# qiyueyao/Kubernetes-verification

Hardware: AMD Instinct MI355X
Metric: pod-pairs/sec for reachability build + all-checks latency, 100k pods, 1/2/4/8 GPU (higher is better)
Workload: dtype u64

## Files before the change

kubernetes-verification_amd/csrc/kano_engine.hpp:

```cpp
#pragma once
#include <hip/hip_runtime.h>
#include <hip/hip_ext.h>

#include <algorithm>
#include <cmath>
#include <functional>
#include <cerrno>
#include <cstdint>
#include <cstdlib>
#include <cstring>
#include <string>
#include <vector>
#include <array>
#include <chrono>
#include <ctime>
#include <cstdio>
#include <dlfcn.h>
#include <link.h>
#include <thread>

#include "kano_hip.h"
#include "kano_internal.hpp"
#include "kano_prims.hpp"

// ... 94 lines not shown
  DBuf mct;
  bool shg_prefilled = false;
  i64 dx_ldY = 0, dx_PBo = 0;
  bool dense_sel = false;
  int ac_lds = 1;
  int mlists_side_ok = 1;
  bool mlists_side = false;
  bool rin_marked = false;
  i64 sel_early_cap = -1;
  int path_lds = 1;
  int rows_ch = ROWS_CH;
  int rows_cww = MAX_CWW_KNOB;
  int impact_form = 0;
  int shadow_r = 0;
  int shg_sub_lds = 1;
  int rows_cu_off = 20;
  int xcd_split = 1;
  i64 xcd_min_bytes = XCD_MIN_BYTES;
  int xcd_write = XCD_WRITE;
  int xcd_eng0 = -1;
  bool xcd_tried = false, eng_on_xcd = false, xcd_last_ok = false;
  int side_mode = 0;
  int xcd_side = -1;
  hipStream_t stream_x = nullptr, stream2_x = nullptr, stream3x = nullptr;
  hipStream_t stream2_u = nullptr;
  hipEvent_t ev_sw = nullptr, ev_sw2 = nullptr;
  i64 rows_cu_bytes = 8ll << 30;
  int num_cus = 0, rows_cus = 0;

  ClassSet rc, cc;
// ... 21 lines not shown
  hipEvent_t ev_pre = nullptr, ev_pre_done = nullptr, ev_pre_ac = nullptr;
  bool pre_forked = false, pre_side_pending = false, pre_ac_pending = false;
  bool tail_compacted = false;
  hipEvent_t ev_pairs = nullptr;
  DBuf gid, gids, cgroup, R, multi, A1, A2, own, cross, gmin, gmax, ckey, corder, kcnt, koff;
  DBuf flags, T, loff, L, tp, poff, out, tcnt, toff;
  DBuf scratch_words, ident;
  DBuf xw, xg;
  i64 xg_emul = -1;
  DBuf pT, pR[2], pD[2], pA, pB, pcnt;
  DBuf xv, asel, aalw, iterm, idead, irows;
  i64 inc_A = 0, inc_acap = 0, inc_xcols = 0;
  std::vector<uint8_t> dead;
  bool user_edited = false;
  i64 shadow_total = -1;
  DBuf conflict_out;
  i64 conflict_total = -1;
  DBuf impact_out, impact_ess;
  float impact_ms = 0.f;
  bool vs_count_only = false;
  bool shg_ran = false;
  DBuf shg_h, shg_tkey, shg_trep, shg_slot, shg_isrep, shg_gidx, shg_gid, shg_reps, shg_sub,
      shg_err;
  DBuf sizes;
  DBuf icnt, ioff, sysrow, idxd;
  u64* ghost = nullptr;
  void* row_stage = nullptr;
  u64* gmirror = nullptr;
  u64* gmirror_dev = nullptr;
  DBuf sig_ctr;
// ... 32 lines not shown
  bool priming = false;
  bool consume_prime = false;
  bool prime_pre_marked = false;
  bool prime_alist_valid = false;
  u64 prime_sig = 0;
  u64* bell = nullptr;
  u64* bell_dev = nullptr;
  u64 bell_seq = 0;
  u64 gate_ticks = 0;
  u64 wall_khz = 100000;
  DBuf gate_wait;
  u64 gate_seq0 = 0;
  u64 gate_forced = 0;
  DBuf sizes_alt;
  hipEvent_t ev_tail = nullptr;
  hipEvent_t ev_rt[2][2] = {};
  bool rows_time_pending[2] = {false, false};
  hipEvent_t ev_m0 = nullptr, ev_m1 = nullptr;
  bool mfma_time_pending = false;
  double mfma_ops_last = 0.0, mfma_ops_sum = 0.0, mfma_ms_sum = 0.0;
  i64 mfma_n = 0;
  float rows_ms_last = 0.f;
  double rows_ms_sum = 0.0, rows_ms_min = 0.0, rows_ms_max = 0.0;
  i64 rows_ms_n = 0;
  bool vs_open = false, vs_shadow = false, vs_cross_want = false, vs_cross_on = false;
  bool vs_have_sys = false, vs_sys_on = false;
  bool vs_rows = false;
  i64 vs_nb = 0, vs_rl = 0;
};

// ... 46 lines not shown
```

kubernetes-verification_amd/csrc/kano_hip.hip:

```cpp
#include "kano_engine.hpp"
#include "kano_kernels.hpp"

namespace kano_eng {

int fail(kano_ctx* ctx, int code, const std::string& msg) {
  ctx->err = msg;
  return code;
}

int settle(kano_ctx* ctx);

int dalloc(kano_ctx* ctx, DBuf& b, size_t bytes) {
  if (bytes == 0) bytes = 16;
  if (b.p && b.bytes >= bytes) return 0;
  if (b.p) {
    KTRY(settle(ctx));
    KCHK(hipFree(b.p));
    b.p = nullptr;
    b.bytes = 0;
  }
  const hipError_t e = hipMalloc(&b.p, bytes);
  if (e != hipSuccess) {
    b.p = nullptr;
    return fail(ctx, -ENOMEM, "hipMalloc(" + std::to_string(bytes) + " bytes) -> " +
// ... 229 lines not shown
  std::swap(ctx->aloff, a.aloff);
  std::swap(ctx->alist, a.alist);
  std::swap(ctx->alcoff, a.alcoff);
  std::swap(ctx->alc, a.alc);
  std::swap(ctx->rc.moff, a.rmoff);
  std::swap(ctx->rc.mem, a.rmem);
  std::swap(ctx->cc.moff, a.cmoff);
  std::swap(ctx->cc.mem, a.cmem);
  std::swap(ctx->cc.cls, a.ccls);
  std::swap(ctx->hflag, a.hflag);
  std::swap(ctx->hlist, a.hlist);
  std::swap(ctx->Mc, a.Mc);
  ctx->rows_set ^= 1;
}

void ring_bell(kano_ctx* ctx) {
  if (ctx->bell) __atomic_store_n(ctx->bell, ctx->bell_seq, __ATOMIC_SEQ_CST);
}

int unprime(kano_ctx* ctx) {
  if (!ctx->primed || ctx->priming) return 0;
  ctx->primed = false;
  ring_bell(ctx);
  ctx->gate_forced = ctx->bell_seq;
  KCHK(hipStreamSynchronize(ctx->stream));
  KCHK(hipStreamSynchronize(ctx->stream2));
  std::swap(ctx->sizes, ctx->sizes_alt);
  swap_rows_ptrs(ctx);
  ctx->alist_valid = ctx->prime_alist_valid;
  return 0;
// ... 62 lines not shown
  KCHK(hipEventElapsedTime(&ms, ctx->ev_m0, ctx->ev_m1));
  ctx->mfma_ms_sum += ms;
  ctx->mfma_ops_sum += ctx->mfma_ops_last;
  ctx->mfma_n += 1;
  return 0;
}

int read_slots(kano_ctx* ctx, int first, int count, i64* out) {
  KCHK(hipMemcpyAsync(ctx->ghost, P_<u64>(ctx->sizes) + first, sizeof(u64) * count,
                      hipMemcpyDeviceToHost, ctx->stream));
  KTRY(sync(ctx));
  for (int k = 0; k < count; ++k) out[k] = (i64)ctx->ghost[k];
  return 0;
}

void* pinned_dev(void* host) {
  if (!host || (reinterpret_cast<uintptr_t>(host) & 15)) return nullptr;
  hipPointerAttribute_t at{};
  void* dptr = nullptr;
  if (hipPointerGetAttributes(&at, host) == hipSuccess && at.type == hipMemoryTypeHost &&
      at.devicePointer)
    dptr = at.devicePointer;
  (void)hipGetLastError();
  return dptr;
}

int copy_out(kano_ctx* ctx, void* host, const void* dev, size_t bytes, hipStream_t st) {
  if (bytes == 0) return 0;
  hipPointerAttribute_t at{};
  void* dptr = nullptr;
  if (hipPointerGetAttributes(&at, host) == hipSuccess && at.type == hipMemoryTypeHost &&
      at.devicePointer)
// ... 306 lines not shown

int sel_spb(const kano_ctx* ctx) {
  return ctx->P >= 8 * std::max<i64>(1, ctx->rc.U) ? TPB : WPB;
}

int front_fills(kano_ctx* ctx, FillBatch& fb) {
  KTRY(dalloc(ctx, ctx->sizes, sizeof(u64) * SZ_SLOTS));
  KTRY(fb.add(ctx->sizes, sizeof(u64) * SZ_SLOTS, 0u));
  KTRY(classify_alloc1(ctx, ctx->rc, fb));
  KTRY(classify_alloc1(ctx, ctx->cc, fb));
  return 0;
}

int select_engine_streams(kano_ctx* ctx);

int front_a(kano_ctx* ctx) {
  KTRY(select_engine_streams(ctx));
  ctx->rc.m0 = ctx->r0;
  ctx->rc.m1 = ctx->r1;
  ctx->cc.m0 = 0;
  ctx->cc.m1 = ctx->n;
  {
    FillBatch fb(ctx);
    KTRY(front_fills(ctx, fb));
    KTRY(fb.run());
  }
  KTRY(classify_phase1(ctx));
  KTRY(mirror_begin(ctx));
  ctx->mlists_side = ctx->stream2 != nullptr && ctx->mlists_side_ok;
  if (!ctx->mlists_side && ctx->stream2) {
    KTRY(classify_phase2a(ctx));
    KCHK(hipEventRecord(ctx->ev_pre, ctx->stream));
    return 0;
  }
  return classify_phase2a(ctx);
}

// ... 1061 lines not shown
        if (k == "packed") ctx->cls_packed = v;
        if (k == "rw" && v >= 0 && v <= 2) ctx->rows_wide = v;
        if (k == "rwg" && v >= 0) ctx->rows_w_grid = v;
        if (k == "rheavy" && v >= 0 && v <= 2) ctx->rows_early_heavy = v;
        if (k == "aipt" && v >= 0 && v <= ASSIGN_IPT) ctx->assign_ipt = v;
        if (k == "sww" && v >= 1 && v <= SORT_LDS_WW) ctx->sort_ww = v;
        if (k == "cww" && v >= 16 && v <= MAX_CWW_KNOB && v % 16 == 0) ctx->rows_cww = v;
        if (k == "rch" && v >= 1 && v <= 1024) ctx->rows_ch = v;
        if (k == "async") ctx->async_rows = v;
        if (k == "shcount" && v >= 0 && v <= 2) ctx->shadow_count_mode = v;
        if (k == "pathdens" && v >= 0 && v <= 101) ctx->path_dens = v;
        if (k == "pathtm" && (v == 1 || v == 2 || v == 4)) ctx->path_tm = v;
        if (k == "pathlds") ctx->path_lds = v;
        if (k == "pathtn" && (v == 2 || v == 4)) ctx->path_tn = v;
        if (k == "shgsub") ctx->shg_sub_lds = v;
        if (k == "impf" && v >= 0 && v <= 2) ctx->impact_form = v;
        if (k == "shr" && (v == 1 || v == 2 || v == 4 || v == 8)) ctx->shadow_r = v;
        if (k == "rcu" && v >= 0 && v <= 28 && (v < 4 || v % 4 == 0)) ctx->rows_cu_off = v;
        if (k == "rcubytes" && v >= 0) ctx->rows_cu_bytes = (i64)v << 30;
        if (k == "xcd") ctx->xcd_split = v;
        if (k == "xcdmin" && v >= 0) ctx->xcd_min_bytes = (i64)v << 10;
        if (k == "xcdw" && v >= 1 && v <= 7) ctx->xcd_write = v;
        if (k == "xcde" && v >= 0 && v <= 7) ctx->xcd_eng0 = v;
        if (k == "xcdside" && v >= -1 && v <= 1) ctx->xcd_side = v;
        if (k == "hgemm" && (v == -1 || v == 0 || v == 22 || v == 42 || v == 44))
          ctx->heavy_gemm = v;
        if (k == "hgemmmin" && v > 0) ctx->heavy_gemm_min = v;
        if (k == "hortime") ctx->time_or = v;
        if (k == "hexplds" && v >= 2 && v <= 4) ctx->heavy_expand_lds = v;
        if (k == "dx") ctx->dx_on = v;
// ... 33 lines not shown
                              hipFuncAttributeMaxDynamicSharedMemorySize,
                              (int)sizeof(u64) * MAX_CWW_KNOB);
  }
  mark("func_attributes");
  if (hipStreamCreateWithFlags(&ctx->stream3, hipStreamNonBlocking) != hipSuccess) {
    ctx->stream3 = nullptr;
    kano_destroy(ctx);
    return -EIO;
  }
  if (!g_create_lean) KTRY(ensure_masked_stream(ctx));
  mark("write_streams");
  if (hipStreamCreateWithPriority(&ctx->stream2, hipStreamNonBlocking, prio_main) != hipSuccess ||
      hipEventCreateWithFlags(&ctx->ev_fork, hipEventDisableTiming) != hipSuccess ||
      hipEventCreateWithFlags(&ctx->ev_sizes, hipEventDisableTiming) != hipSuccess ||
      hipEventCreateWithFlags(&ctx->ev_tail, hipEventDisableTiming) != hipSuccess ||
      hipEventCreateWithFlags(&ctx->ev_rin, hipEventDisableTiming) != hipSuccess ||
      hipEventCreateWithFlags(&ctx->ev_rin_e, hipEventDisableTiming) != hipSuccess ||
      hipEventCreateWithFlags(&ctx->ev_fork2, hipEventDisableTiming) != hipSuccess ||
      hipEventCreateWithFlags(&ctx->ev_join2, hipEventDisableTiming) != hipSuccess ||
      hipEventCreateWithFlags(&ctx->ev_pre, hipEventDisableTiming) != hipSuccess ||
      hipEventCreateWithFlags(&ctx->ev_pre_done, hipEventDisableTiming) != hipSuccess ||
      hipEventCreateWithFlags(&ctx->ev_pre_ac, hipEventDisableTiming) != hipSuccess ||
      hipEventCreateWithFlags(&ctx->ev_sw, hipEventDisableTiming) != hipSuccess ||
      hipEventCreateWithFlags(&ctx->ev_sw2, hipEventDisableTiming) != hipSuccess ||
      hipEventCreateWithFlags(&ctx->ev_pairs, hipEventDisableTiming) != hipSuccess ||
      hipEventCreate(&ctx->ev_m0) != hipSuccess || hipEventCreate(&ctx->ev_m1) != hipSuccess ||
      hipEventCreateWithFlags(&ctx->ev_rows_end[0], hipEventDisableTiming) != hipSuccess ||
      hipEventCreateWithFlags(&ctx->ev_rows_end[1], hipEventDisableTiming) != hipSuccess ||
      hipEventCreate(&ctx->ev_rt[0][0]) != hipSuccess || hipEventCreate(&ctx->ev_rt[0][1]) != hipSuccess ||
      hipEventCreate(&ctx->ev_rt[1][0]) != hipSuccess || hipEventCreate(&ctx->ev_rt[1][1]) != hipSuccess) {
    kano_destroy(ctx);
// ... 95 lines not shown
  RowsInputs& ra = ctx->rin_alt;
  for (DBuf* b : {&ra.wioff, &ra.wicls, &ra.soffc, &ra.slist, &ra.aloff, &ra.alist, &ra.alcoff,
                  &ra.alc, &ra.rmoff, &ra.rmem, &ra.cmoff, &ra.cmem, &ra.ccls, &ra.hflag,
                  &ra.hlist, &ra.Mc})
    dfree(*b);
  for (auto& e : ctx->ev)
    if (e) (void)hipEventDestroy(e);
  if (ctx->own_stream && ctx->stream) (void)hipStreamDestroy(ctx->stream);
  if (ctx->stream2) (void)hipStreamDestroy(ctx->stream2);
  if (ctx->stream3) (void)hipStreamDestroy(ctx->stream3);
  if (ctx->stream3m) (void)hipStreamDestroy(ctx->stream3m);
  for (hipStream_t t : {ctx->stream_x, ctx->stream2_x, ctx->stream3x, ctx->stream2_u})
    if (t) (void)hipStreamDestroy(t);
  for (hipEvent_t e : {ctx->ev_sw, ctx->ev_sw2})
    if (e) (void)hipEventDestroy(e);
  for (hipEvent_t e : {ctx->ev_fork, ctx->ev_tail, ctx->ev_rin, ctx->ev_rin_e, ctx->ev_sizes,
                       ctx->ev_fork2, ctx->ev_join2, ctx->ev_pre, ctx->ev_pre_done, ctx->ev_pre_ac, ctx->ev_pairs, ctx->ev_m0, ctx->ev_m1, ctx->ev_rows_end[0],
                       ctx->ev_rows_end[1], ctx->ev_rt[0][0], ctx->ev_rt[0][1], ctx->ev_rt[1][0],
                       ctx->ev_rt[1][1]})
    if (e) (void)hipEventDestroy(e);
  delete ctx;
}

const char* kano_last_error(const kano_ctx* ctx) { return ctx ? ctx->err.c_str() : "null context"; }

int kano_set_stream(kano_ctx* ctx, void* s) {
  if (!ctx) return -EINVAL;
  KCHK(hipSetDevice(ctx->device));
  KTRY(settle(ctx));
  KTRY(leave_xcd_streams(ctx));
  KCHK(hipStreamSynchronize(ctx->stream2));
// ... 292 lines not shown
               const PreRun& pre_run = PreRun()) {
  if (!ctx) return -EINVAL;
  const bool consume = ctx->primed && ctx->consume_prime;
  ctx->consume_prime = false;
  if (!consume) KTRY(unprime(ctx));
  if (!ctx->have_pods || !ctx->have_pols) return fail(ctx, -EINVAL, "kano_build: inputs not set");
  if (path < 0 || path > 2) return fail(ctx, -EINVAL, "kano_build: unknown path");
  KCHK(hipSetDevice(ctx->device));
  ctx->built = false;
  ctx->rows_deferred = false;
  ctx->lists_mode = false;
  ctx->rows_timed = false;
  ctx->rows_dirty = false;
  ctx->cols_valid = false;
  ctx->shadow_total = -1;
  ctx->conflict_total = -1;
  ctx->sig_armed = 0;
  ctx->sel_early_cap = -1;
  ctx->shg_prefilled = false;
  const i64 rl = rows_local(ctx);
  if (!ctx->defer_alloc)
    KTRY(dalloc(ctx, ctx->M, sizeof(u64) * std::max<i64>(1, rl * ctx->ldM)));
  KTRY(dalloc(ctx, ctx->color, sizeof(u64) * ctx->ldM));
  KTRY(dalloc(ctx, ctx->colnand, sizeof(u64) * ctx->ldM));
  KTRY(stage_mark(ctx, 0, ctx->stream));
  KTRY(do_front(ctx, path, consume));
  KTRY(mirror_begin(ctx));
  KTRY(do_back_pre(ctx, pre_fill, pre_run));
  KTRY(sel_place_early(ctx));
  KTRY(read_sizes(ctx));
// ... 474 lines not shown
  if (nt > 0 && nl > 0) {
    hipLaunchKernelGGL(k_shadow_compact, dim3((unsigned)nt), dim3(TPB), 0, st,
                       P_<i64>(ctx->soffc), U, P_<int32_t>(ctx->slist), P_<i64>(ctx->pfoff),
                       P_<uint8_t>(ctx->flags), nf, P_<i64>(ctx->toff), P_<int2>(ctx->L), nl);
    KLAUNCH();
  }
  if (rl > 0 && total > 0) {
    hipLaunchKernelGGL(k_shadow_emit, dim3(nblk(rl)), dim3(TPB), 0, st,
                       P_<int32_t>(ctx->rc.cls), ctx->r0, ctx->r1, P_<i64>(ctx->loff),
                       P_<int2>(ctx->L), P_<i64>(ctx->poff), P_<int2>(ctx->out), total,
                       (const i64*)nullptr, nl);
    KLAUNCH();
  }
  KTRY(stage_mark(ctx, 6, st));
  ctx->shadow_total = total;
  return 0;
}

}

extern "C" {

int kano_shadow(kano_ctx* ctx, int64_t* count) {
  KTRY(ensure_built(ctx));
  ctx->vs_count_only = false;
  KTRY(shadow_front(ctx));
  i64 tot[2] = {0, 0};
  KTRY(read_slots(ctx, SZ_NL, 2, tot));
  KTRY(shadow_back(ctx, tot[0], tot[1]));
  if (count) *count = tot[1];
  return 0;
}

int kano_shadow_fetch(kano_ctx* ctx, int32_t* pairs) {
  KTRY(ensure_built(ctx));
  if (ctx->shadow_total < 0) return fail(ctx, -EINVAL, "kano_shadow_fetch before kano_shadow");
  if (ctx->shadow_total > 0) {
    if (!pairs) return fail(ctx, -EINVAL, "kano_shadow_fetch: NULL buffer");
    KCHK(hipMemcpyAsync(pairs, ctx->out.p, sizeof(int2) * ctx->shadow_total,
                        hipMemcpyDeviceToHost, ctx->stream));
  }
  return sync(ctx);
}

}

namespace {
int lists_setup(kano_ctx* ctx, const char* what, int64_t n_lists, int64_t nbits, int64_t P,
                const int64_t* soff, const int32_t* slist, const uint64_t* allow_rows) {
  if (!ctx) return -EINVAL;
  if (n_lists < 0 || nbits < 0 || P < 0 || !soff || n_lists >= (int64_t)INT32_MAX / 2)
    return fail(ctx, -EINVAL, std::string(what) + ": bad arguments");
  KCHK(hipSetDevice(ctx->device));
  KTRY(settle(ctx));
  const i64 nnz = soff[n_lists];
  for (i64 e = 0; e < nnz; ++e)
    if (slist[e] < 0 || slist[e] >= P)
      return fail(ctx, -ERANGE, std::string(what) + ": policy index out of range");
  ctx->conflict_total = -1;
  ctx->built = false;
  ctx->lists_mode = true;
  ctx->n = nbits;
  ctx->W = (nbits + 63) / 64;
  ctx->ldM = std::max<i64>(2, (ctx->W + 1) & ~(i64)1);
  ctx->P = P;
  ctx->PB = (P + 63) / 64;
  ctx->r0 = 0;
  ctx->r1 = n_lists;
  ctx->nnz_sel = nnz;
// ... 67 lines not shown
  return kano_shadow(ctx, count);
}

int kano_conflict(kano_ctx* ctx, int* raises) {
  KTRY(ensure_built(ctx));
  if (!raises) return fail(ctx, -EINVAL, "kano_conflict: NULL");
  *raises = ctx->max_sel >= 2 ? 1 : 0;
  return 0;
}

}

namespace {
int conflict_front(kano_ctx* ctx, bool count_only, i64* nl, i64* total) {
  ShadowPlan sp;
  sp.U = ctx->rc.U;
  sp.rl = rows_local(ctx);
  sp.nf = ctx->nflags;
  sp.nt = (sp.nf + SH_TILE - 1) / SH_TILE;
  KTRY(dalloc(ctx, ctx->sizes, sizeof(u64) * SZ_SLOTS));
  KTRY(dalloc(ctx, ctx->flags, count_only ? 16 : 8 * ((sp.nf + 63) / 64) + 16));
  KTRY(dalloc(ctx, ctx->T, sizeof(i64) * std::max<i64>(1, sp.U)));
  KTRY(dalloc(ctx, ctx->loff, sizeof(i64) * (sp.U + 1)));
  KTRY(dalloc(ctx, ctx->tp, sizeof(i64) * std::max<i64>(1, sp.rl)));
  KTRY(dalloc(ctx, ctx->poff, sizeof(i64) * (sp.rl + 1)));
  {
    FillBatch fb(ctx);
    if (!count_only) {
      KTRY(dalloc(ctx, ctx->tcnt, sizeof(i64) * std::max<i64>(1, sp.nt)));
      KTRY(dalloc(ctx, ctx->toff, sizeof(i64) * (sp.nt + 1)));
// ... 438 lines not shown
    if (q != hipErrorNotReady) KCHK(q);
    __builtin_ia32_pause();
    if ((spin & 0xff) == 0 && clk::now() - t0 > std::chrono::seconds(1)) {
      KCHK(hipEventSynchronize(e));
      return 0;
    }
  }
}

int prime_next(kano_ctx* ctx) {
  if (ctx->primed || !ctx->bell || ctx->stage_timing) return 0;
  KTRY(dalloc(ctx, ctx->sizes_alt, sizeof(u64) * SZ_SLOTS));
  ctx->prime_alist_valid = ctx->alist_valid;
  KTRY(swap_rows_inputs(ctx));
  std::swap(ctx->sizes, ctx->sizes_alt);
  ctx->primed = true;
  ctx->priming = true;
  const u64 armed = ctx->sig_armed, waiting = ctx->sig_wait;
  if (!ctx->gate_wait.p) {
    KTRY(dalloc(ctx, ctx->gate_wait, sizeof(u64) * GATE_RING));
    KCHK(hipMemsetAsync(ctx->gate_wait.p, 0, sizeof(u64) * GATE_RING, ctx->stream));
  }
  hipLaunchKernelGGL(k_gate, dim3(1), dim3(64), 0, ctx->stream, (const u64*)ctx->bell_dev,
                     ++ctx->bell_seq, ctx->gate_ticks, P_<u64>(ctx->gate_wait));
  int rc = hipGetLastError() == hipSuccess ? 0 : fail(ctx, -EIO, "k_gate launch failed");
  if (!rc) {
    ctx->sig_armed = 0;
    rc = front_a(ctx);
  }
  ctx->priming = false;
  if (rc) {
    (void)unprime(ctx);
    return rc;
  }
  ctx->prime_sig = ctx->sig_wait;
  ctx->sig_armed = armed;
  ctx->sig_wait = waiting;
  return 0;
}

int verify_back_direct(kano_ctx* ctx, int32_t* idx, void* idx_h, int64_t* counts,
                       int32_t* shadow_pairs, void* pairs_h, int64_t shadow_cap,
                       int64_t* shadow_count, bool async, bool compacted = false) {
  using clk = std::chrono::steady_clock;
  auto tmark = clk::now();
  auto part = [&](int k) {
    const auto t = clk::now();
    ctx->ht[k] = std::max(ctx->ht[k], std::chrono::duration<double, std::micro>(t - tmark).count());
    tmark = t;
  };
  const i64 n = ctx->n, rl = ctx->vs_rl;
  const bool want_shadow = ctx->vs_shadow;
  const bool pairs_mode = want_shadow && shadow_cap >= 0;
  hipStream_t st = ctx->stream;
  const i64 nf = ctx->nflags, nt = (nf + SH_TILE - 1) / SH_TILE;
  i64 out_cap = 0;
  const bool pairs_job = pairs_mode && pairs_h && rl > 0;
  const u64* tots = P_<u64>(ctx->sizes) + SZ_IDX0;
  if (pairs_mode) {
    KTRY(dalloc(ctx, ctx->L, sizeof(int2) * std::max<i64>(1, nf)));
    KTRY(dalloc(ctx, ctx->out, sizeof(int2) * 1024));
    out_cap = (i64)(ctx->out.bytes / sizeof(int2));
    if (compacted) KCHK(hipStreamWaitEvent(st, ctx->ev_pairs, 0));
    if (nt > 0 && !compacted) {
      hipLaunchKernelGGL(k_shadow_compact, dim3((unsigned)nt), dim3(TPB), 0, st,
                         P_<i64>(ctx->soffc), ctx->rc.U, P_<int32_t>(ctx->slist),
                         P_<i64>(ctx->pfoff), P_<uint8_t>(ctx->flags), nf, P_<i64>(ctx->toff),
                         P_<int2>(ctx->L), nf);
      KLAUNCH();
    }
    if (rl > 0) {
      hipLaunchKernelGGL(k_shadow_emit, dim3(nblk(rl)), dim3(TPB), 0, st,
                         P_<int32_t>(ctx->rc.cls), ctx->r0, ctx->r1, P_<i64>(ctx->loff),
                         P_<int2>(ctx->L), P_<i64>(ctx->poff), P_<int2>(ctx->out), out_cap,
                         nt > 0 ? P_<i64>(ctx->toff) + nt : (const i64*)nullptr, nf);
      KLAUNCH();
    }
  }
  CopySegs cj{};
  int njobs = 0;
  cj.j[njobs++] = CopySeg{static_cast<const char*>(ctx->idxd.p), static_cast<char*>(idx_h),
                          tots, 4, nullptr, 0, 4, 4 * n};
  if (pairs_job) {
    cj.j[njobs++] = CopySeg{static_cast<const char*>(ctx->out.p), static_cast<char*>(pairs_h),
                            reinterpret_cast<const u64*>(P_<i64>(ctx->poff) + rl), 1, nullptr, 0,
                            8, std::min<i64>(shadow_cap, out_cap)};
  }
  if (njobs > 0) {
    hipExtLaunchKernelGGL(k_copy_segs, dim3(256, njobs), dim3(TPB), 0, st, nullptr, ctx->ev_tail,
                          0, cj);
    KLAUNCH();
  }
  if (ctx->vs_rows) {
    ctx->rows_overlap = async;
    ctx->rows_in = ctx->rin_marked ? ctx->ev_rin_e : ctx->ev_tail;
    ctx->rin_marked = false;
    const int rc = launch_rows(ctx);
    ctx->rows_overlap = false;
    ctx->rows_in = nullptr;
    KTRY(rc);
  }
  if (async && ctx->pipeline) KTRY(prime_next(ctx));
  part(12);
  const auto tw0 = clk::now();
  KTRY(spin_event(ctx, ctx->ev_tail));
  ctx->ht[18] += std::chrono::duration<double, std::micro>(clk::now() - tw0).count();
  part(14);
  ctx->sig_wait = 0;
  constexpr int NS = SZ_ERR - SZ_NL + 1;
  i64 v[NS];
  for (int q = 0; q < NS; ++q) v[q] = (i64)((volatile u64*)ctx->gmirror)[SZ_NL + q];
  if (ctx->vs_cross_on && (v[SZ_ERR - SZ_NL] & 0xffffffff)) {
    (void)settle(ctx);
    (void)sync(ctx);
    return fail(ctx, -EINVAL, "kano_verify: a group id lies outside [0, ngroups)");
  }
  for (int r = 0; r < 4; ++r) counts[r] = v[SZ_IDX0 - SZ_NL + r];
  if (!ctx->vs_have_sys) counts[3] = -1;
  if (want_shadow) {
    const i64 total = v[SZ_PAIRS - SZ_NL];
    *shadow_count = total;
    ctx->shadow_total = pairs_mode ? total : -1;
    if (pairs_mode && total > out_cap) {
      KTRY(unprime(ctx));
      KTRY(dalloc(ctx, ctx->out, sizeof(int2) * (total + total / 4)));
      if (rl > 0) {
        hipLaunchKernelGGL(k_shadow_emit, dim3(nblk(rl)), dim3(TPB), 0, st,
                           P_<int32_t>(ctx->rc.cls), ctx->r0, ctx->r1, P_<i64>(ctx->loff),
                           P_<int2>(ctx->L), P_<i64>(ctx->poff), P_<int2>(ctx->out), total,
                           (const i64*)nullptr, nf);
        KLAUNCH();
      }
      if (shadow_pairs && total <= shadow_cap)
        KTRY(copy_out(ctx, shadow_pairs, ctx->out.p, sizeof(int2) * total, st));
      KCHK(hipEventRecord(ctx->ev_tail, st));
      KCHK(hipEventSynchronize(ctx->ev_tail));
    }
  }
// ... 8 lines not shown

int verify_back(kano_ctx* ctx, const u64* gathered, int32_t nranks, int32_t* idx, int64_t* counts,
                int32_t* shadow_pairs, int64_t shadow_cap, int64_t* shadow_count,
                bool may_async = false) {
  if (!ctx->vs_open) return fail(ctx, -EINVAL, "kano_verify_combine without kano_verify_shard");
  ctx->vs_open = false;
  const i64 n = ctx->n, W = ctx->W, nb = ctx->vs_nb;
  const bool want_shadow = ctx->vs_shadow;
  const bool cross_row = gathered ? ctx->vs_cross_want : ctx->vs_cross_on;
  const bool pairs_mode = want_shadow && shadow_cap >= 0;
  if (want_shadow && ctx->vs_count_only && shadow_cap >= 0) {
    (void)sync(ctx);
    return fail(ctx, -EINVAL, "kano_verify_combine: the shard ran policy_shadow count-only "
                              "(with_shadow = 2); pass shadow_cap < 0");
  }
  void* idx_h = n > 0 ? pinned_dev(idx) : nullptr;
  void* pairs_h = pairs_mode && shadow_pairs ? pinned_dev(shadow_pairs) : nullptr;
  const bool direct = n > 0 && W > 0 && idx_h && (!pairs_mode || !shadow_pairs || pairs_h);
  const bool side_sh = want_shadow && ctx->tail_compacted;
  const bool compacted = side_sh && direct && pairs_mode;
  if (side_sh && !compacted) KCHK(hipStreamWaitEvent(ctx->stream, ctx->ev_pairs, 0));
  ctx->tail_compacted = false;
  ScanBatch sb(ctx);
  if (want_shadow && !side_sh)
    KTRY(sb.add(P_<i64>(ctx->tp), ctx->vs_rl, P_<i64>(ctx->poff), SZ_PAIRS));
  if (gathered && n > 0 && W > 0) {
    if (cross_row) KTRY(dalloc(ctx, ctx->cross, sizeof(u64) * ctx->ldM));
    hipLaunchKernelGGL(k_combine_cols, dim3((unsigned)nb), dim3(TPB), 0, ctx->stream, gathered,
                       nranks, n, W, nb, P_<u64>(ctx->color), P_<u64>(ctx->colnand),
                       P_<u64>(ctx->col_and), cross_row ? P_<u64>(ctx->cross) : nullptr,
                       P_<i64>(ctx->icnt));
    KLAUNCH();
  }
  for (int r = 0; r < 4; ++r)
    KTRY(sb.add(P_<i64>(ctx->icnt) + r * nb, nb, P_<i64>(ctx->ioff) + r * (nb + 1),
                SZ_IDX0 + r));
  sb.publish(SZ_ERR);
  if (want_shadow && !compacted) sb.publish(SZ_NL);
  if (sb.jobs.count == 0) ctx->sig_armed = 0;
  KTRY(sb.run());
  IdxRows ir{};
  ir.W = W;
  ir.n = n;
  ir.nb = nb;
  ir.row[0] = P_<u64>(ctx->col_and);
  ir.row[1] = P_<u64>(ctx->color);
  ir.inv[1] = 1;
  ir.row[2] = cross_row ? P_<u64>(ctx->cross) : nullptr;
  ir.row[3] = ctx->vs_sys_on ? P_<u64>(ctx->sysrow) : nullptr;
  ir.inv[3] = 1;
  int32_t* idx_dev = P_<int32_t>(ctx->idxd);
  if (n > 0 && W > 0) {
    hipLaunchKernelGGL(k_idx_write, dim3((unsigned)nb, 4), dim3(TPB), 0, ctx->stream, ir,
                       P_<i64>(ctx->ioff), nb + 1, P_<u64>(ctx->sizes) + SZ_IDX0, idx_dev);
    KLAUNCH();
  }
  if (direct)
    return verify_back_direct(ctx, idx, idx_h, counts, shadow_pairs, pairs_h, shadow_cap,
                              shadow_count, may_async && ctx->async_rows, compacted);
  constexpr int NS = SZ_ERR - SZ_NL + 1;
  using clk = std::chrono::steady_clock;
  auto tmark = clk::now();
  auto part = [&](int k) {
    const auto t = clk::now();
    ctx->ht[k] = std::max(ctx->ht[k], std::chrono::duration<double, std::micro>(t - tmark).count());
    tmark = t;
  };
  const bool signalled = ctx->sig_armed != 0;
  KTRY(mirror_begin(ctx));
  hipEvent_t tail_ev = signalled ? nullptr : ctx->ev_sizes;
  const bool async = may_async && ctx->async_rows;
  if (!tail_ev) {
    KCHK(hipEventRecord(ctx->ev_sizes, ctx->stream));
    tail_ev = ctx->ev_sizes;
// ... 391 lines not shown
```

kubernetes-verification_amd/csrc/kano_kernels.hpp:

```cpp
#pragma once
#include "kano_prims.hpp"

namespace kano {

struct ClsSide {
  const int32_t* keys;
  int KS;
  int packed;
  int pbits;
  uint32_t tmask;
  int32_t* table;
  int32_t* slot_of;
  int32_t* smin;
  int32_t* flag;
  const int32_t* cid;
  int32_t* cls;
  int32_t* rep;
  int32_t* mcnt;
  int32_t* mcur;
  const int32_t* moff;
  int32_t* mem;
  int32_t* cval;
  i64 m0, m1, U;
};
// ... 3132 lines not shown
__global__ __launch_bounds__(TPB) void k_idx_write(IdxRows a, const i64* __restrict__ boff,
                                                   i64 ldo, const u64* __restrict__ rowtot,
                                                   int32_t* __restrict__ idx) {
  __shared__ i64 sm[4];
  const int r = blockIdx.y;
  const i64 j = (i64)blockIdx.x * TPB + threadIdx.x;
  bool bit = false;
  if (a.row[r] && j < a.n) bit = ((a.row[r][j >> 6] >> (j & 63)) & 1ull) != (a.inv[r] != 0);
  i64 row0 = 0;
  for (int q = 0; q < r; ++q) row0 += (i64)rowtot[q];
  i64 tot;
  const i64 pos = block_excl_scan((i64)bit, sm, tot) + row0 + boff[r * ldo + blockIdx.x];
  if (bit) idx[pos] = (int32_t)j;
}

}
```

Measured before the change: 31600 billion.

## Fuse verify tail scan, index write and pair emit into one direct-to-host kernel

When the block count is small, the separate scan batch, k_idx_write, k_shadow_emit and k_copy_segs steps are replaced by one k_tail_fused kernel. It computes offsets by summing icnt per block, stages the selected indices in LDS and writes them and the shadow pairs straight into pinned host memory, while also publishing row totals to the host mirror. Pair emission can optionally run split onto a second stream. The device-side shadow output buffer is now rebuilt lazily when it is later fetched, and fills plus buffer presizing move ahead of the gate during priming. The aim is fewer launches and less serial latency in the tail, at the cost of redundant per-block prefix sums and more complex staleness handling.

```diff
diff --git a/kubernetes-verification_amd/csrc/kano_engine.hpp b/kubernetes-verification_amd/csrc/kano_engine.hpp
--- a/kubernetes-verification_amd/csrc/kano_engine.hpp
+++ b/kubernetes-verification_amd/csrc/kano_engine.hpp
@@ -132,6 +132,9 @@
   int impact_form = 0;
   int shadow_r = 0;
   int shg_sub_lds = 1;
+  i64 tail_fused_nb = 1024;
+  int tail_split = 1;
+  int pregate_fills = 1;
   int rows_cu_off = 20;
   int xcd_split = 1;
   i64 xcd_min_bytes = XCD_MIN_BYTES;
@@ -183,6 +186,7 @@
   std::vector<uint8_t> dead;
   bool user_edited = false;
   i64 shadow_total = -1;
+  bool out_stale = false;
   DBuf conflict_out;
   i64 conflict_total = -1;
   DBuf impact_out, impact_ess;
@@ -245,6 +249,7 @@
   u64 gate_forced = 0;
   DBuf sizes_alt;
   hipEvent_t ev_tail = nullptr;
+  hipEvent_t ev_tail2 = nullptr;
   hipEvent_t ev_rt[2][2] = {};
   bool rows_time_pending[2] = {false, false};
   hipEvent_t ev_m0 = nullptr, ev_m1 = nullptr;
diff --git a/kubernetes-verification_amd/csrc/kano_hip.hip b/kubernetes-verification_amd/csrc/kano_hip.hip
--- a/kubernetes-verification_amd/csrc/kano_hip.hip
+++ b/kubernetes-verification_amd/csrc/kano_hip.hip
@@ -267,6 +267,20 @@
   ctx->rows_set ^= 1;
 }
 
+int presize_rows_inputs(kano_ctx* ctx) {
+  RowsInputs& a = ctx->rin_alt;
+  DBuf* const cur[] = {&ctx->wioff,  &ctx->wicls,   &ctx->soffc,   &ctx->slist, &ctx->aloff,
+                       &ctx->alist,  &ctx->alcoff,  &ctx->alc,     &ctx->rc.moff, &ctx->rc.mem,
+                       &ctx->cc.moff, &ctx->cc.mem, &ctx->cc.cls,  &ctx->hflag, &ctx->hlist,
+                       &ctx->Mc};
+  const DBuf* const last[] = {&a.wioff, &a.wicls,  &a.soffc, &a.slist, &a.aloff, &a.alist,
+                              &a.alcoff, &a.alc,   &a.rmoff, &a.rmem,  &a.cmoff, &a.cmem,
+                              &a.ccls,  &a.hflag,  &a.hlist, &a.Mc};
+  for (size_t k = 0; k < sizeof(cur) / sizeof(cur[0]); ++k)
+    if (last[k]->bytes > cur[k]->bytes) KTRY(dalloc(ctx, *cur[k], last[k]->bytes));
+  return 0;
+}
+
 void ring_bell(kano_ctx* ctx) {
   if (ctx->bell) __atomic_store_n(ctx->bell, ctx->bell_seq, __ATOMIC_SEQ_CST);
 }
@@ -359,8 +373,8 @@
   return 0;
 }
 
-void* pinned_dev(void* host) {
-  if (!host || (reinterpret_cast<uintptr_t>(host) & 15)) return nullptr;
+void* pinned_dev(void* host, size_t align) {
+  if (!host || (reinterpret_cast<uintptr_t>(host) & (align - 1))) return nullptr;
   hipPointerAttribute_t at{};
   void* dptr = nullptr;
   if (hipPointerGetAttributes(&at, host) == hipSuccess && at.type == hipMemoryTypeHost &&
@@ -697,13 +711,13 @@
 
 int select_engine_streams(kano_ctx* ctx);
 
-int front_a(kano_ctx* ctx) {
+int front_a(kano_ctx* ctx, bool filled = false) {
   KTRY(select_engine_streams(ctx));
   ctx->rc.m0 = ctx->r0;
   ctx->rc.m1 = ctx->r1;
   ctx->cc.m0 = 0;
   ctx->cc.m1 = ctx->n;
-  {
+  if (!filled) {
     FillBatch fb(ctx);
     KTRY(front_fills(ctx, fb));
     KTRY(fb.run());
@@ -1795,6 +1809,9 @@
         if (k == "pathlds") ctx->path_lds = v;
         if (k == "pathtn" && (v == 2 || v == 4)) ctx->path_tn = v;
         if (k == "shgsub") ctx->shg_sub_lds = v;
+        if (k == "tfnb" && v >= 0) ctx->tail_fused_nb = v;
+        if (k == "pregate") ctx->pregate_fills = v;
+        if (k == "tsplit" && v >= 0 && v <= 2) ctx->tail_split = v;
         if (k == "impf" && v >= 0 && v <= 2) ctx->impact_form = v;
         if (k == "shr" && (v == 1 || v == 2 || v == 4 || v == 8)) ctx->shadow_r = v;
         if (k == "rcu" && v >= 0 && v <= 28 && (v < 4 || v % 4 == 0)) ctx->rows_cu_off = v;
@@ -1858,7 +1875,8 @@
       hipEventCreateWithFlags(&ctx->ev_fork, hipEventDisableTiming) != hipSuccess ||
       hipEventCreateWithFlags(&ctx->ev_sizes, hipEventDisableTiming) != hipSuccess ||
       hipEventCreateWithFlags(&ctx->ev_tail, hipEventDisableTiming) != hipSuccess ||
-      hipEventCreateWithFlags(&ctx->ev_rin, hipEventDisableTiming) != hipSuccess ||
+      hipEventCreateWithFlags(&ctx->ev_tail2, hipEventDisableTiming) != hipSuccess ||
+      hipEventCreateWithFlags(&ctx->ev_rin,hipEventDisableTiming) != hipSuccess ||
       hipEventCreateWithFlags(&ctx->ev_rin_e, hipEventDisableTiming) != hipSuccess ||
       hipEventCreateWithFlags(&ctx->ev_fork2, hipEventDisableTiming) != hipSuccess ||
       hipEventCreateWithFlags(&ctx->ev_join2, hipEventDisableTiming) != hipSuccess ||
@@ -1984,7 +2002,7 @@
     if (t) (void)hipStreamDestroy(t);
   for (hipEvent_t e : {ctx->ev_sw, ctx->ev_sw2})
     if (e) (void)hipEventDestroy(e);
-  for (hipEvent_t e : {ctx->ev_fork, ctx->ev_tail, ctx->ev_rin, ctx->ev_rin_e, ctx->ev_sizes,
+  for (hipEvent_t e : {ctx->ev_fork, ctx->ev_tail, ctx->ev_tail2, ctx->ev_rin, ctx->ev_rin_e, ctx->ev_sizes,
                        ctx->ev_fork2, ctx->ev_join2, ctx->ev_pre, ctx->ev_pre_done, ctx->ev_pre_ac, ctx->ev_pairs, ctx->ev_m0, ctx->ev_m1, ctx->ev_rows_end[0],
                        ctx->ev_rows_end[1], ctx->ev_rt[0][0], ctx->ev_rt[0][1], ctx->ev_rt[1][0],
                        ctx->ev_rt[1][1]})
@@ -2307,6 +2325,7 @@
   ctx->rows_dirty = false;
   ctx->cols_valid = false;
   ctx->shadow_total = -1;
+  ctx->out_stale = false;
   ctx->conflict_total = -1;
   ctx->sig_armed = 0;
   ctx->sel_early_cap = -1;
@@ -2811,6 +2830,21 @@
   }
   KTRY(stage_mark(ctx, 6, st));
   ctx->shadow_total = total;
+  ctx->out_stale = false;
+  return 0;
+}
+
+int shadow_out_refresh(kano_ctx* ctx) {
+  if (!ctx->out_stale) return 0;
+  ctx->out_stale = false;
+  const i64 total = ctx->shadow_total, rl = rows_local(ctx);
+  if (total <= 0 || rl <= 0) return 0;
+  KTRY(dalloc(ctx, ctx->out, sizeof(int2) * total));
+  hipLaunchKernelGGL(k_shadow_emit, dim3(nblk(rl)), dim3(TPB), 0, ctx->stream,
+                     P_<int32_t>(ctx->rc.cls), ctx->r0, ctx->r1, P_<i64>(ctx->loff),
+                     P_<int2>(ctx->L), P_<i64>(ctx->poff), P_<int2>(ctx->out), total,
+                     (const i64*)nullptr, ctx->nflags);
+  KLAUNCH();
   return 0;
 }
 
@@ -2832,6 +2866,7 @@
 int kano_shadow_fetch(kano_ctx* ctx, int32_t* pairs) {
   KTRY(ensure_built(ctx));
   if (ctx->shadow_total < 0) return fail(ctx, -EINVAL, "kano_shadow_fetch before kano_shadow");
+  KTRY(shadow_out_refresh(ctx));
   if (ctx->shadow_total > 0) {
     if (!pairs) return fail(ctx, -EINVAL, "kano_shadow_fetch: NULL buffer");
     KCHK(hipMemcpyAsync(pairs, ctx->out.p, sizeof(int2) * ctx->shadow_total,
@@ -2850,6 +2885,7 @@
     return fail(ctx, -EINVAL, std::string(what) + ": bad arguments");
   KCHK(hipSetDevice(ctx->device));
   KTRY(settle(ctx));
+  KTRY(shadow_out_refresh(ctx));
   const i64 nnz = soff[n_lists];
   for (i64 e = 0; e < nnz; ++e)
     if (slist[e] < 0 || slist[e] >= P)
@@ -2947,6 +2983,7 @@
 namespace {
 int conflict_front(kano_ctx* ctx, bool count_only, i64* nl, i64* total) {
   ShadowPlan sp;
+  KTRY(shadow_out_refresh(ctx));
   sp.U = ctx->rc.U;
   sp.rl = rows_local(ctx);
   sp.nf = ctx->nflags;
@@ -3415,19 +3452,38 @@
   ctx->prime_alist_valid = ctx->alist_valid;
   KTRY(swap_rows_inputs(ctx));
   std::swap(ctx->sizes, ctx->sizes_alt);
+  int rc = presize_rows_inputs(ctx);
+  if (!rc && !ctx->gate_wait.p) {
+    rc = dalloc(ctx, ctx->gate_wait, sizeof(u64) * GATE_RING);
+    if (!rc && hipMemsetAsync(ctx->gate_wait.p, 0, sizeof(u64) * GATE_RING, ctx->stream) !=
+                   hipSuccess)
+      rc = fail(ctx, -EIO, "gate ring reset failed");
+  }
+  const bool filled = ctx->pregate_fills != 0;
+  if (!rc && filled) {
+    ctx->rc.m0 = ctx->r0;
+    ctx->rc.m1 = ctx->r1;
+    ctx->cc.m0 = 0;
+    ctx->cc.m1 = ctx->n;
+    FillBatch fb(ctx);
+    rc = front_fills(ctx, fb);
+    if (!rc) rc = fb.run();
+  }
+  if (rc) {
+    std::swap(ctx->sizes, ctx->sizes_alt);
+    swap_rows_ptrs(ctx);
+    ctx->alist_valid = ctx->prime_alist_valid;
+    return rc;
+  }
   ctx->primed = true;
   ctx->priming = true;
   const u64 armed = ctx->sig_armed, waiting = ctx->sig_wait;
-  if (!ctx->gate_wait.p) {
-    KTRY(dalloc(ctx, ctx->gate_wait, sizeof(u64) * GATE_RING));
-    KCHK(hipMemsetAsync(ctx->gate_wait.p, 0, sizeof(u64) * GATE_RING, ctx->stream));
-  }
   hipLaunchKernelGGL(k_gate, dim3(1), dim3(64), 0, ctx->stream, (const u64*)ctx->bell_dev,
                      ++ctx->bell_seq, ctx->gate_ticks, P_<u64>(ctx->gate_wait));
-  int rc = hipGetLastError() == hipSuccess ? 0 : fail(ctx, -EIO, "k_gate launch failed");
+  rc = hipGetLastError() == hipSuccess ? 0 : fail(ctx, -EIO, "k_gate launch failed");
   if (!rc) {
     ctx->sig_armed = 0;
-    rc = front_a(ctx);
+    rc = front_a(ctx, filled);
   }
   ctx->priming = false;
   if (rc) {
@@ -3442,7 +3498,8 @@
 
 int verify_back_direct(kano_ctx* ctx, int32_t* idx, void* idx_h, int64_t* counts,
                        int32_t* shadow_pairs, void* pairs_h, int64_t shadow_cap,
-                       int64_t* shadow_count, bool async, bool compacted = false) {
+                       int64_t* shadow_count, bool async, bool compacted = false,
+                       const IdxRows* fused = nullptr, bool publish_nl = false) {
   using clk = std::chrono::steady_clock;
   auto tmark = clk::now();
   auto part = [&](int k) {
@@ -3457,12 +3514,16 @@
   const i64 nf = ctx->nflags, nt = (nf + SH_TILE - 1) / SH_TILE;
   i64 out_cap = 0;
   const bool pairs_job = pairs_mode && pairs_h && rl > 0;
+  const bool split = fused && compacted && pairs_job &&
+                     (ctx->tail_split == 2 || (ctx->tail_split == 1 && rl == n));
   const u64* tots = P_<u64>(ctx->sizes) + SZ_IDX0;
   if (pairs_mode) {
     KTRY(dalloc(ctx, ctx->L, sizeof(int2) * std::max<i64>(1, nf)));
-    KTRY(dalloc(ctx, ctx->out, sizeof(int2) * 1024));
-    out_cap = (i64)(ctx->out.bytes / sizeof(int2));
-    if (compacted) KCHK(hipStreamWaitEvent(st, ctx->ev_pairs, 0));
+    if (!fused) {
+      KTRY(dalloc(ctx, ctx->out, sizeof(int2) * 1024));
+      out_cap = (i64)(ctx->out.bytes / sizeof(int2));
+    }
+    if (compacted && !split) KCHK(hipStreamWaitEvent(st, ctx->ev_pairs, 0));
     if (nt > 0 && !compacted) {
       hipLaunchKernelGGL(k_shadow_compact, dim3((unsigned)nt), dim3(TPB), 0, st,
                          P_<i64>(ctx->soffc), ctx->rc.U, P_<int32_t>(ctx->slist),
@@ -3470,7 +3531,7 @@
                          P_<int2>(ctx->L), nf);
       KLAUNCH();
     }
-    if (rl > 0) {
+    if (rl > 0 && !fused) {
       hipLaunchKernelGGL(k_shadow_emit, dim3(nblk(rl)), dim3(TPB), 0, st,
                          P_<int32_t>(ctx->rc.cls), ctx->r0, ctx->r1, P_<i64>(ctx->loff),
                          P_<int2>(ctx->L), P_<i64>(ctx->poff), P_<int2>(ctx->out), out_cap,
@@ -3478,16 +3539,55 @@
       KLAUNCH();
     }
   }
-  CopySegs cj{};
-  int njobs = 0;
-  cj.j[njobs++] = CopySeg{static_cast<const char*>(ctx->idxd.p), static_cast<char*>(idx_h),
-                          tots, 4, nullptr, 0, 4, 4 * n};
-  if (pairs_job) {
-    cj.j[njobs++] = CopySeg{static_cast<const char*>(ctx->out.p), static_cast<char*>(pairs_h),
-                            reinterpret_cast<const u64*>(P_<i64>(ctx->poff) + rl), 1, nullptr, 0,
-                            8, std::min<i64>(shadow_cap, out_cap)};
-  }
-  if (njobs > 0) {
+  if (fused) {
+    TailArgs ta{};
+    ta.ir = *fused;
+    ta.icnt = P_<i64>(ctx->icnt);
+    ta.idx_h = static_cast<int32_t*>(idx_h);
+    ta.nlb = (fused->nb + TAIL_G - 1) / TAIL_G;
+    if (pairs_job) {
+      ta.npb = nblk(rl);
+      ta.cls = P_<int32_t>(ctx->rc.cls);
+      ta.r0 = ctx->r0;
+      ta.r1 = ctx->r1;
+      ta.loff = P_<i64>(ctx->loff);
+      ta.L = P_<int2>(ctx->L);
+      ta.poff = P_<i64>(ctx->poff);
+      ta.pairs_h = static_cast<int2*>(pairs_h);
+      ta.pairs_cap = shadow_cap;
+    }
+    ta.rowtot = P_<u64>(ctx->sizes) + SZ_IDX0;
+    ta.rowtot_host = ctx->gmirror_dev + SZ_IDX0;
+    ta.pub_src[ta.npub] = P_<u64>(ctx->sizes) + SZ_ERR;
+    ta.pub_dst[ta.npub++] = ctx->gmirror_dev + SZ_ERR;
+    if (publish_nl) {
+      ta.pub_src[ta.npub] = P_<u64>(ctx->sizes) + SZ_NL;
+      ta.pub_dst[ta.npub++] = ctx->gmirror_dev + SZ_NL;
+    }
+    if (split) {
+      TailArgs tp = ta;
+      tp.nlb = 0;
+      tp.rowtot = nullptr;
+      tp.npub = 0;
+      hipExtLaunchKernelGGL(k_tail_fused, dim3((unsigned)tp.npb), dim3(TPB), 0, ctx->stream2,
+                            nullptr, ctx->ev_tail2, 0, tp);
+      KLAUNCH();
+      ta.npb = 0;
+    }
+    hipExtLaunchKernelGGL(k_tail_fused,
+                          dim3((unsigned)(4 * ta.nlb + ta.npb + (ta.rowtot ? 1 : 0))), dim3(TPB),
+                          0, st, nullptr, ctx->ev_tail, 0, ta);
+    KLAUNCH();
+  } else {
+    CopySegs cj{};
+    int njobs = 0;
+    cj.j[njobs++] = CopySeg{static_cast<const char*>(ctx->idxd.p), static_cast<char*>(idx_h),
+                            tots, 4, nullptr, 0, 4, 4 * n};
+    if (pairs_job) {
+      cj.j[njobs++] = CopySeg{static_cast<const char*>(ctx->out.p), static_cast<char*>(pairs_h),
+                              reinterpret_cast<const u64*>(P_<i64>(ctx->poff) + rl), 1, nullptr, 0,
+                              8, std::min<i64>(shadow_cap, out_cap)};
+    }
     hipExtLaunchKernelGGL(k_copy_segs, dim3(256, njobs), dim3(TPB), 0, st, nullptr, ctx->ev_tail,
                           0, cj);
     KLAUNCH();
@@ -3505,6 +3605,7 @@
   part(12);
   const auto tw0 = clk::now();
   KTRY(spin_event(ctx, ctx->ev_tail));
+  if (split) KTRY(spin_event(ctx, ctx->ev_tail2));
   ctx->ht[18] += std::chrono::duration<double, std::micro>(clk::now() - tw0).count();
   part(14);
   ctx->sig_wait = 0;
@@ -3522,7 +3623,8 @@
     const i64 total = v[SZ_PAIRS - SZ_NL];
     *shadow_count = total;
     ctx->shadow_total = pairs_mode ? total : -1;
-    if (pairs_mode && total > out_cap) {
+    ctx->out_stale = fused && pairs_mode;
+    if (!fused && pairs_mode && total > out_cap) {
       KTRY(unprime(ctx));
       KTRY(dalloc(ctx, ctx->out, sizeof(int2) * (total + total / 4)));
       if (rl > 0) {
@@ -3561,8 +3663,8 @@
     return fail(ctx, -EINVAL, "kano_verify_combine: the shard ran policy_shadow count-only "
                               "(with_shadow = 2); pass shadow_cap < 0");
   }
-  void* idx_h = n > 0 ? pinned_dev(idx) : nullptr;
-  void* pairs_h = pairs_mode && shadow_pairs ? pinned_dev(shadow_pairs) : nullptr;
+  void* idx_h = n > 0 ? pinned_dev(idx, sizeof(int32_t)) : nullptr;
+  void* pairs_h = pairs_mode && shadow_pairs ? pinned_dev(shadow_pairs, sizeof(int2)) : nullptr;
   const bool direct = n > 0 && W > 0 && idx_h && (!pairs_mode || !shadow_pairs || pairs_h);
   const bool side_sh = want_shadow && ctx->tail_compacted;
   const bool compacted = side_sh && direct && pairs_mode;
@@ -3579,11 +3681,14 @@
                        P_<i64>(ctx->icnt));
     KLAUNCH();
   }
-  for (int r = 0; r < 4; ++r)
-    KTRY(sb.add(P_<i64>(ctx->icnt) + r * nb, nb, P_<i64>(ctx->ioff) + r * (nb + 1),
-                SZ_IDX0 + r));
-  sb.publish(SZ_ERR);
-  if (want_shadow && !compacted) sb.publish(SZ_NL);
+  const bool fused = direct && ctx->gmirror_dev && nb <= ctx->tail_fused_nb;
+  if (!fused) {
+    for (int r = 0; r < 4; ++r)
+      KTRY(sb.add(P_<i64>(ctx->icnt) + r * nb, nb, P_<i64>(ctx->ioff) + r * (nb + 1),
+                  SZ_IDX0 + r));
+    sb.publish(SZ_ERR);
+    if (want_shadow && !compacted) sb.publish(SZ_NL);
+  }
   if (sb.jobs.count == 0) ctx->sig_armed = 0;
   KTRY(sb.run());
   IdxRows ir{};
@@ -3597,14 +3702,15 @@
   ir.row[3] = ctx->vs_sys_on ? P_<u64>(ctx->sysrow) : nullptr;
   ir.inv[3] = 1;
   int32_t* idx_dev = P_<int32_t>(ctx->idxd);
-  if (n > 0 && W > 0) {
+  if (n > 0 && W > 0 && !fused) {
     hipLaunchKernelGGL(k_idx_write, dim3((unsigned)nb, 4), dim3(TPB), 0, ctx->stream, ir,
                        P_<i64>(ctx->ioff), nb + 1, P_<u64>(ctx->sizes) + SZ_IDX0, idx_dev);
     KLAUNCH();
   }
   if (direct)
     return verify_back_direct(ctx, idx, idx_h, counts, shadow_pairs, pairs_h, shadow_cap,
-                              shadow_count, may_async && ctx->async_rows, compacted);
+                              shadow_count, may_async && ctx->async_rows, compacted,
+                              fused ? &ir : nullptr, want_shadow && !compacted);
   constexpr int NS = SZ_ERR - SZ_NL + 1;
   using clk = std::chrono::steady_clock;
   auto tmark = clk::now();
diff --git a/kubernetes-verification_amd/csrc/kano_kernels.hpp b/kubernetes-verification_amd/csrc/kano_kernels.hpp
--- a/kubernetes-verification_amd/csrc/kano_kernels.hpp
+++ b/kubernetes-verification_amd/csrc/kano_kernels.hpp
@@ -3170,4 +3170,119 @@
   if (bit) idx[pos] = (int32_t)j;
 }
 
-}
+constexpr int TAIL_G = 4;
+struct TailArgs {
+  IdxRows ir;
+  const i64* icnt;
+  int32_t* idx_h;
+  i64 nlb, npb;
+  const int32_t* cls;
+  i64 r0, r1;
+  const i64* loff;
+  const int2* L;
+  const i64* poff;
+  int2* pairs_h;
+  i64 pairs_cap;
+  u64* rowtot;
+  u64* rowtot_host;
+  int npub;
+  const u64* pub_src[2];
+  u64* pub_dst[2];
+};
+
+__global__ __launch_bounds__(TPB) void k_tail_fused(TailArgs a) {
+  __shared__ i64 sm[4];
+  __shared__ int32_t stage[TAIL_G * TPB];
+  __shared__ int s_rel[TPB];
+  __shared__ i64 s_l0[TPB];
+  const int tid = threadIdx.x;
+  const i64 nb = a.ir.nb;
+  const i64 blk = blockIdx.x;
+  if (blk < 4 * a.nlb) {
+    const int r = (int)(blk / a.nlb);
+    const i64 b0 = (blk - (i64)r * a.nlb) * TAIL_G;
+    i64 s = 0;
+    for (i64 i = tid, e = (i64)r * nb + b0; i < e; i += TPB) s += a.icnt[i];
+    const i64 off = block_sum(s, sm);
+    const u64* row = a.ir.row[r];
+    const bool inv = a.ir.inv[r] != 0;
+    int run = 0;
+    for (int g = 0; g < TAIL_G && b0 + g < nb; ++g) {
+      const i64 j = (b0 + g) * TPB + tid;
+      bool bit = false;
+      if (row && j < a.ir.n) bit = (((row[j >> 6] >> (j & 63)) & 1ull) != 0) != inv;
+      i64 tot;
+      const i64 p = block_excl_scan((i64)bit, sm, tot);
+      if (bit) stage[run + (int)p] = (int32_t)j;
+      run += (int)tot;
+    }
+    __syncthreads();
+    int32_t* dst = a.idx_h + off;
+    const int head =
+        min(run, (int)(((16 - (reinterpret_cast<uintptr_t>(dst) & 15)) & 15) >> 2));
+    if (tid < head) dst[tid] = stage[tid];
+    const int n16 = (run - head) >> 2;
+    uint4* d16 = reinterpret_cast<uint4*>(dst + head);
+    for (int k = tid; k < n16; k += TPB) {
+      const int32_t* sp = stage + head + 4 * k;
+      d16[k] = make_uint4((uint32_t)sp[0], (uint32_t)sp[1], (uint32_t)sp[2], (uint32_t)sp[3]);
+    }
+    const int t0 = head + 4 * n16;
+    if (tid < run - t0) dst[t0 + tid] = stage[t0 + tid];
+    return;
+  }
+  if (blk < 4 * a.nlb + a.npb) {
+    const i64 rl = a.r1 - a.r0;
+    if (a.poff[rl] > a.pairs_cap) return;
+    const i64 wb = a.r0 + (blk - 4 * a.nlb) * TPB;
+    const i64 we = min(wb + TPB, a.r1), i = wb + tid;
+    const i64 ob = a.poff[wb - a.r0], oe = a.poff[we - a.r0];
+    i64 l0 = 0, o = oe;
+    if (i < we) {
+      l0 = a.loff[a.cls[i]];
+      o = a.poff[i - a.r0];
+    }
+    if (oe - ob > (i64)INT32_MAX) {
+      if (i < we)
+        for (i64 k = 0, len = a.poff[i + 1 - a.r0] - o; k < len; ++k) a.pairs_h[o + k] = a.L[l0 + k];
+      return;
+    }
+    const int tot = (int)(oe - ob);
+    s_rel[tid] = (int)(o - ob);
+    s_l0[tid] = l0;
+    __syncthreads();
+    auto pair_at = [&](int q) {
+      int j = 0;
+#pragma unroll
+      for (int st = TPB / 2; st >= 1; st >>= 1)
+        if (s_rel[j + st] <= q) j += st;
+      return a.L[s_l0[j] + (q - s_rel[j])];
+    };
+    static_assert(TPB == 256, "the search covers indices 0..255 from 0 in steps 128..1");
+    int2* dst = a.pairs_h + ob;
+    const int head = min(tot, (int)((reinterpret_cast<uintptr_t>(dst) & 15) >> 3));
+    if (tid == 0 && head) dst[0] = pair_at(0);
+    const int n16 = (tot - head) >> 1;
+    uint4* d16 = reinterpret_cast<uint4*>(dst + head);
+    for (int k = tid; k < n16; k += TPB) {
+      const int2 p0 = pair_at(head + 2 * k), p1 = pair_at(head + 2 * k + 1);
+      d16[k] = make_uint4((uint32_t)p0.x, (uint32_t)p0.y, (uint32_t)p1.x, (uint32_t)p1.y);
+    }
+    if (tid == 0 && ((tot - head) & 1)) dst[tot - 1] = pair_at(tot - 1);
+    return;
+  }
+  if (!a.rowtot) return;
+  for (int r = 0; r < 4; ++r) {
+    i64 s = 0;
+    for (i64 i = tid; i < nb; i += TPB) s += a.icnt[(i64)r * nb + i];
+    const i64 t = block_sum(s, sm);
+    if (tid == 0) {
+      a.rowtot[r] = (u64)t;
+      if (a.rowtot_host) mirror_store(a.rowtot_host + r, (u64)t);
+    }
+  }
+  if (tid == 0)
+    for (int q = 0; q < a.npub; ++q) mirror_store(a.pub_dst[q], *a.pub_src[q]);
+}
+
+}
```

After: 31540 billion. About the same (-0.2%).
